# namascar/correlation

Hardware: AMD Instinct MI355X
Metric: correlation-point-iterations/sec (higher is better)
Workload: dtype f32

## Files before the change

### correlation_amd/csrc/lk_device.hpp

```cpp
#pragma once
#include <hip/hip_runtime.h>
#include <stdint.h>

#include "../../include/lk_engine.h"

struct LkLevelView {
  const uint8_t *und;
  const uint8_t *def;
  const float2 *xy;
  const float2 *xy_eval;
  const uint32_t *off;
  const int4 *rect;
  int urows, ucols;
  int drows, dcols;
};

struct LkHandoff {
  float p[6];
  int level;
  int level_old;
  int reached;
  uint32_t n_evals, n_sample_evals, n_point_iters;
};

struct LkSeqFrame {
  const uint8_t *und[LK_MAX_LEVELS];
  const uint8_t *def[LK_MAX_LEVELS];
};
constexpr int kLkSeqChainWords = 16;

constexpr int kLkMaxTeam = 256;
constexpr int kLkMidWords = 32;

struct LkSolveArgs {
  const LkLevelView *lv;
  const float2 *center;
  const float *guess;
  lk_result *result;
  float *last_p;
  float *last_eval_p;
  uint32_t *stats;
  const uint32_t *order;
  int team_w;
  int team_min_samples;
  float *team_partials;
  uint32_t *team_arrivals;
  int team_fault;
  int eval_cap;
  int finisher;
  int resume;
  uint32_t *ill_list;
  uint32_t *ill_count;
  uint32_t *mid_state;
  uint32_t *finish_list;
  uint32_t *finish_count;
  LkHandoff *handoff;
  uint32_t *queue;
  int n_sectors;
  int chunk;
  int align;
  int solo;
  int safe;
  int reference_order;
  int mark_stale;
  int persistent;
  int rows_used;
  int starved_max;
  int keep_sums;
  int gpu_share;
  int slots_permille;
  int py_start, py_step, py_stop;
  float precision;
  int max_iters;
  int seq_frames;
  int seq_velocity;
  int seq_stride;
  const LkSeqFrame *seq_img;
  unsigned long long *seq_chain;
  const float *seq_prev_p;
  float *seq_prev_p_out;
  float *seq_guess_out;
  uint32_t *seq_flags;
  const uint32_t *seq_gate;
  int seq_fault;
};

struct LkRoiSector {
  int kind;
  int x0, y0, x1, y1;
  float cx, cy, ri2, ro2;
  float q00x, q01x, q10x, q11x, q00y, q01y, q10y, q11y;
  int as;
  int flat_begin, flat_count;
};
struct LkRoiFlat {
  float ls, li, rs, ri;
  int j0, j1;
  int row_begin;
};
constexpr int kLkRoiTile = 1024;

struct LkRewarpArgs {
  const float2 *src_xy;
  const uint32_t *src_off;
  const int4 *src_rect;
  const uint32_t *dst_off;
  float2 *dst_xy;
  const float2 *center;
  const float *p;
  const float2 *offset;
  int n_sectors;
  uint32_t total;
  int rows;
};

struct LkAppendArgs {
  int sector, n_levels;
  int keep_state;
  float2 center;
  float2 *d_center;
  float *d_guess, *d_last_p, *d_prev_p, *d_last_eval_p;
  lk_result *d_result;
  uint32_t *d_stats;
  int4 rect[LK_MAX_LEVELS];
  uint32_t off_end[LK_MAX_LEVELS];
  int4 *d_rect[LK_MAX_LEVELS];
  uint32_t *d_off[LK_MAX_LEVELS];
};

struct LkEvalArgs {
  const LkLevelView *lv;
  const float2 *center;
  int sector, level;
  float p[6];
  float *out;
  int ref_threads;
};

struct LkGuessSearchArgs {
  const uint8_t *und, *def;
  int urows, ucols, drows, dcols;
  const float2 *xy;
  const uint32_t *off;
  const int4 *rect;
  float *guess;
  float *prev_p;
  lk_guess_match *match;
  int n_sectors, level, radius, has_v, min_samples;
  float min_score;
  int win_bytes;
};
constexpr int kLkGsThreads = 256;
constexpr int kLkGsChunk = 1024;

struct LkBackwardArgs {
  const LkLevelView *lv;
  const float2 *center;
  const float *guess;
  lk_result *result;
  float *last_p;
  float *last_eval_p;
  uint32_t *stats;
  const uint32_t *order;
  float4 *tpl;
  const uint32_t *tpl_base;
  int n_sectors;
  int py_start, py_step, py_stop;
// ... 16 lines not shown
```

### correlation_amd/csrc/lk_engine.cpp

```cpp
#include "lk_compose.hpp"
#include "lk_device.hpp"
#include "lk_internal.hpp"
#include "lk_roi.hpp"

#include <rocprofiler-sdk-roctx/roctx.h>

#include <algorithm>
#include <chrono>
#include <climits>
#include <cstdio>
#include <cstdlib>
#include <cstring>
#include <functional>
#include <mutex>
#include <string>
#include <thread>
#include <vector>

hipError_t lk_launch_solve(const LkSolveArgs &a, int model, int interp, int group, hipStream_t st);
hipError_t lk_launch_solve_seq(const LkSolveArgs &a, int model, int interp, int group, int flavour, hipStream_t st);
hipError_t lk_launch_eval(const LkEvalArgs &a, int model, int interp, int group, hipStream_t st);
hipError_t lk_launch_solve_only(int n, const float *d_in, float *d_out, hipStream_t st);
hipError_t lk_launch_step_compare(int n, const float *d_in, float *d_out, hipStream_t st);
hipError_t lk_launch_reduce_compare(int n, int wide, const float *d_in, float *d_out, hipStream_t st);
// ... 862 lines not shown
    for (int k = w; k < count; k += workers) {
      const float *q = params + 6 * (size_t)k;
      HostSector &s = e->hs[(size_t)(first_sector + k)];
      s.xy.clear();
      s.is_rect = false;
      s.flats.clear();
      s.fresh = true;
      if (!lkroi::annular_geometry(q[0], q[1], q[2], q[3], q[4], q[5], as, s.ag)) {
        empty[(size_t)w] = 1;
        continue;
      }
      s.lazy = 1;
      if (on_host) {
        s.realize();
        if (s.xy.empty()) {
          empty[(size_t)w] = 1;
          continue;
        }
      }
      s.has_center = false;
      s.set = true;
    }
  };
  std::vector<std::thread> th;
  for (int w = 1; w < workers; ++w)
    th.emplace_back(work, w);
  work(0);
  for (std::thread &t : th)
    t.join();
  for (int v : empty)
    if (v)
      return e->fail(LK_ERROR_BAD_DOMAIN, "lk_set_sectors_annular: empty sector");
  return LK_ERROR_NONE;
}

int lk_set_sector_blob(lk_engine *e, int sector, const float *contour_xy, int n_vertices) {
  if (!e)
    return LK_ERROR_BAD_DOMAIN;
  HostSector *s = sector_slot(e, sector);
  if (!s || !contour_xy)
    return e->fail(LK_ERROR_BAD_DOMAIN, "lk_set_sector_blob: bad arguments");
  s->xy.clear();
  s->is_rect = false;
  s->flats.clear();
  s->lazy = 0;
  if (host_roi()) {
    if (!lkroi::BlobPolygon::inside_points(contour_xy, n_vertices, s->xy) || s->xy.empty()) {
      s->set = false;
      return e->fail(LK_ERROR_BAD_DOMAIN, "lk_set_sector_blob: contour is not a simple polygon");
    }
    lkroi::mean_center(s->xy.data(), (int)(s->xy.size() / 2), s->cx, s->cy);
  } else {
    if (!lkroi::BlobPolygon::flat_triangles(contour_xy, n_vertices, s->flats) || s->flats.empty()) {
      s->set = false;
      return e->fail(LK_ERROR_BAD_DOMAIN, "lk_set_sector_blob: contour is not a simple polygon");
    }
    s->lazy = 2;
  }
  s->has_center = false;
  s->set = true;
  return LK_ERROR_NONE;
}

int lk_set_sector_points(lk_engine *e, int sector, const float *xy, int n, int use_center, float cx,
                         float cy) {
  if (!e)
    return LK_ERROR_BAD_DOMAIN;
  HostSector *s = sector_slot(e, sector);
  if (!s || !xy || n < 1)
    return e->fail(LK_ERROR_BAD_DOMAIN, "lk_set_sector_points: bad arguments");
  s->xy.assign(xy, xy + 2 * (size_t)n);
  s->is_rect = false;
  if (use_center) {
    s->cx = cx;
    s->cy = cy;
  } else {
    lkroi::mean_center(xy, n, s->cx, s->cy);
  }
  s->has_center = use_center != 0;
  s->set = true;
  return LK_ERROR_NONE;
}

static int starved_max(const lk_engine *e) { return e->starved_max >= 0 ? e->starved_max : 2 * e->P; }
static int refresh_starved(lk_engine *e) {
  const int S = (int)e->h_class.size();
  {
    const char *f = std::getenv("LK_STARVED_MAX");
    e->starved_max = f ? std::atoi(f) : -1;
  }
  for (int c = 0; c < kNumClasses; ++c)
    e->class_starved[c] = false;
  if (const char *f = std::getenv("LK_FORCE_SAFE"))
    e->force_safe = std::atoi(f) != 0;
  const int l = e->cfg.py_stop;
  bool any_starved = false;
  for (int s = 0; s < S; ++s) {
    const int4 r = e->h_rect[l][(size_t)s];
    const int n = r.z > 0 ? r.w : (int)(e->h_off[l][(size_t)s + 1] - e->h_off[l][(size_t)s]);
    if (n <= starved_max(e))
      e->class_starved[e->h_class[(size_t)s]] = any_starved = true;
  }
  if (any_starved) {
    HIPCHK(e->d_finish_list.ensure((size_t)S));
    HIPCHK(e->d_finish_count.ensure(kNumClasses));
  }
  return LK_ERROR_NONE;
}

static int level0_count(const lk_engine *e, int s) {
  const int4 r = e->h_rect[0][(size_t)s];
  return r.z > 0 ? r.w : (int)(e->h_off[0][(size_t)s + 1] - e->h_off[0][(size_t)s]);
}

static int build_lists_roi_device(lk_engine *e, const std::vector<int> &levels) {
  Range range_("lk:roi masks");
  const int S = (int)e->hs.size();
  hipStream_t st = e->stream;
  std::vector<LkRoiSector> sec((size_t)S);
  std::vector<LkRoiFlat> flats;
  std::vector<uint32_t> tile_begin((size_t)S + 1, 0u);
  uint64_t tiles = 0;
  bool non_negative = true;
  for (int s = 0; s < S; ++s) {
    const HostSector &h = e->hs[(size_t)s];
    LkRoiSector &q = sec[(size_t)s];
    std::memset(&q, 0, sizeof(q));
    tile_begin[(size_t)s] = (uint32_t)tiles;
    if (h.lazy == 1) {
      const lkroi::AnnularGeometry &g = h.ag;
      q.kind = 0;
      q.x0 = g.x0, q.y0 = g.y0, q.x1 = g.x1, q.y1 = g.y1;
      q.cx = g.cx, q.cy = g.cy, q.ri2 = g.ri2, q.ro2 = g.ro2;
      q.q00x = g.q00x, q.q01x = g.q01x, q.q10x = g.q10x, q.q11x = g.q11x;
      q.q00y = g.q00y, q.q01y = g.q01y, q.q10y = g.q10y, q.q11y = g.q11y;
      q.as = g.as;
      const int64_t w = std::max(0, g.x1 - g.x0), hh = std::max(0, g.y1 - g.y0);
      if (w * hh >= (int64_t)1 << 31)
        return e->fail(LK_ERROR_BAD_DOMAIN, "lk_commit_sectors: annular sector bounding box too large");
      q.x1 = q.x0 + (int)w, q.y1 = q.y0 + (int)hh;
      non_negative = non_negative && std::max((float)q.x0, g.cx - g.ro) >= 0.f && std::max((float)q.y0, g.cy - g.ro) >= 0.f &&
                     q.x1 < (1 << 15) && q.y1 < (1 << 15);
      tiles += (uint64_t)((w * hh + kLkRoiTile - 1) / kLkRoiTile);
    } else {
      q.kind = 1;
      q.flat_begin = (int)flats.size();
      q.flat_count = (int)h.flats.size();
      uint64_t rows = 0;
      for (const lkroi::BlobPolygon::Flat &f : h.flats) {
        LkRoiFlat d;
        d.ls = f.ls, d.li = f.li, d.rs = f.rs, d.ri = f.ri, d.j0 = f.j0, d.j1 = f.j1;
        d.row_begin = (int)rows;
        rows += (uint64_t)(f.j1 - f.j0);
        flats.push_back(d);
        for (int j : {f.j0, f.j1 - 1}) {
          const float a = std::ceil(f.ls * (float)j + f.li), b = std::ceil(f.rs * (float)j + f.ri);
          non_negative = non_negative && j >= 0 && j < (1 << 15) && a >= 0.f && b < 32768.f;
        }
      }
      tiles += rows;
    }
    if (tiles >= (uint64_t)1 << 31)
      return e->fail(LK_ERROR_BAD_DOMAIN, "lk_commit_sectors: region of interest too large for the device mask");
  }
  tile_begin[(size_t)S] = (uint32_t)tiles;
  const uint32_t n_tiles = (uint32_t)tiles;
  if (n_tiles == 0)
    return e->fail(LK_ERROR_BAD_DOMAIN, "lk_commit_sectors: empty region of interest");
  HIPCHK(e->d_roi_sectors.ensure((size_t)S));
  HIPCHK(e->d_roi_flats.ensure(flats.size() + 1));
  HIPCHK(e->d_roi_tile_begin.ensure((size_t)S + 1));
  HIPCHK(hipMemcpyAsync(e->d_roi_sectors.p, sec.data(), (size_t)S * sizeof(LkRoiSector), hipMemcpyHostToDevice, st));
// ... 1023 lines not shown
  if (!xy || cap <= 0)
    return LK_ERROR_NONE;
  HIPCHK(hipSetDevice(e->cfg.device));
  HIPCHK(e->d_warp.ensure(2 * (size_t)n));
  HIPCHK(hipMemcpyAsync(e->d_warp.p + n, pts.data(), 2 * sizeof(float) * (size_t)n, hipMemcpyHostToDevice,
                        e->stream));
  float pp[6] = {0, 0, 0, 0, 0, 0};
  for (int i = 0; i < e->P; ++i)
    pp[i] = p[i];
  HIPCHK(hipMemcpyAsync(e->d_scratch.p, pp, sizeof(pp), hipMemcpyHostToDevice, e->stream));
  HIPCHK(lk_launch_warp_points(e->d_warp.p + n, n, e->h_center[2 * (size_t)sector],
                               e->h_center[2 * (size_t)sector + 1], e->cfg.fitting_model, e->d_scratch.p,
                               e->d_warp.p, e->stream));
  HIPCHK(hipMemcpyAsync(xy, e->d_warp.p, 2 * sizeof(float) * (size_t)std::min(n, cap),
                        hipMemcpyDeviceToHost, e->stream));
  HIPCHK(hipStreamSynchronize(e->stream));
  return LK_ERROR_NONE;
}

static int refresh_level_views(lk_engine *e) {
  if (!e->committed)
    return e->fail(LK_ERROR_BAD_DOMAIN, "sectors are not committed (call lk_commit_sectors)");
  if (e->recommit_pending) {
    e->recommit_pending = false;
    int rc = commit_impl(e, true);
    if (rc)
      return rc;
  }
  const DevImage &u = e->img[LK_IMG_UND], &d = e->img[LK_IMG_DEF];
  if (!u.valid || !d.valid)
    return e->fail(LK_ERROR_BAD_DOMAIN, "undeformed and deformed images must be set before correlating");
  if (!e->lv_dirty)
    return LK_ERROR_NONE;
  for (int l = 0; l < LK_MAX_LEVELS; ++l) {
    LkLevelView &v = e->h_lv[l];
    std::memset(&v, 0, sizeof(v));
    if (l > e->cfg.py_stop)
      continue;
    v.und = u.lvl[l];
    v.def = d.lvl[l];
    v.xy = e->d_xy[l].p;
    v.xy_eval = e->eval_lists && !e->batch_invariant ? e->d_xy_eval[l].p : nullptr;
    v.off = e->d_off[l].p;
    v.rect = e->d_rect[l].p;
    v.urows = u.rows >> l;
    v.ucols = u.cols >> l;
    v.drows = d.rows >> l;
    v.dcols = d.cols >> l;
  }
  if (!e->d_lv.p || std::memcmp(e->h_lv, e->h_lv_sent, sizeof(e->h_lv)) != 0) {
    HIPCHK(e->d_lv.ensure(LK_MAX_LEVELS));
    HIPCHK(lk_launch_set_views(e->h_lv, e->d_lv.p, e->stream));
    std::memcpy(e->h_lv_sent, e->h_lv, sizeof(e->h_lv));
  }
  e->lv_dirty = false;
  return LK_ERROR_NONE;
}

static bool safe_flavour(const lk_engine *e) { return e->force_safe || e->batch_invariant; }

static LkSolveArgs base_args(lk_engine *e, const float *d_guess, lk_result *d_result) {
  LkSolveArgs a{};
  a.lv = e->d_lv.p;
  a.center = e->d_center.p;
  a.guess = d_guess;
  a.result = d_result;
  a.last_p = e->d_last_p.p;
  a.last_eval_p = e->d_last_eval_p.p;
  a.stats = e->d_stats.p;
  a.py_start = e->cfg.py_start;
  a.py_step = e->cfg.py_step;
  a.py_stop = e->cfg.py_stop;
  a.precision = e->cfg.precision;
  a.max_iters = e->cfg.max_iters;
  a.solo = e->batch_invariant ? 0 : 1;
  a.gpu_share = e->pairs_in_flight;
  static const int align = [] {
    const char *f = std::getenv("LK_ALIGN");
    return f ? std::atoi(f) : 1;
  }();
  a.align = align;
  const char *ks = std::getenv("LK_KEEP_SUMS");
  a.keep_sums = ks ? (std::atoi(ks) != 0 ? 1 : 0) : 1;
  a.starved_max = starved_max(e);
  return a;
}

static int launch_starved(lk_engine *e, LkSolveArgs &a, int c, int first, hipStream_t st) {
  a.handoff = e->d_handoff.p;
  a.eval_cap = e->eval_cap > 0 ? e->eval_cap : 0;
  a.mid_state = e->d_mid.p;
  a.finish_list = e->d_finish_list.p + first;
  a.finish_count = e->d_finish_count.p + c;
  if (a.eval_cap > 0)
    HIPCHK(hipMemsetAsync(a.finish_count, 0, sizeof(uint32_t), st));
  HIPCHK(lk_launch_solve(a, e->cfg.fitting_model, e->cfg.interpolation, 1, st));
  if (a.eval_cap > 0) {
    LkSolveArgs f = a;
    f.finisher = 1;
    f.safe = 1;
    f.align = 0;
    HIPCHK(lk_launch_solve(f, e->cfg.fitting_model, e->cfg.interpolation, 16, st));
  }
  a.eval_cap = 0;
  return LK_ERROR_NONE;
}

static int launch_groups(lk_engine *e, LkSolveArgs &a, int group, int c, int first, hipStream_t st) {
  static const bool ill_env = [] { const char *f = std::getenv("LK_ILL_PASS"); return f ? std::atoi(f) != 0 : true; }();
  const bool with_ill_pass = !a.safe && ill_env;
  if (with_ill_pass) {
    a.mid_state = e->d_mid.p;
    a.ill_list = e->d_ill_list.p + first;
    a.ill_count = e->d_ill_count.p + c;
  }
  HIPCHK(lk_launch_solve(a, e->cfg.fitting_model, e->cfg.interpolation, group, st));
  if (with_ill_pass) {
    LkSolveArgs r = a;
    r.resume = 1;
    r.safe = 1;
    r.ill_list = nullptr;
    r.ill_count = nullptr;
    r.finish_list = a.ill_list;
    r.finish_count = a.ill_count;
    r.team_w = 0;
    r.handoff = nullptr;
    r.queue = a.queue + 3;
    HIPCHK(lk_launch_solve(r, e->cfg.fitting_model, e->cfg.interpolation, 16, st));
  }
  return LK_ERROR_NONE;
}

static int team_fault_hook() {
  const char *f = std::getenv("LK_TEAM_FAULT");
  return f ? std::atoi(f) : 0;
}
static std::mutex g_team_mu;
static hipEvent_t g_team_done[64] = {};

static int stale_iterations(lk_engine *e, lk_result *d_result, int n) {
  if (!e->d_stale.p) {
    HIPCHK(e->d_stale.ensure(2));
    HIPCHK(hipMemsetAsync(e->d_stale.p, 0, 2 * sizeof(int), e->stream));
  }
  HIPCHK(lk_launch_stale_iterations(d_result, n, e->d_stale.p + e->stale_par, e->d_stale.p + (e->stale_par ^ 1), e->stream));
  e->stale_par ^= 1;
  return LK_ERROR_NONE;
}

static const int kBwGroups[3] = {16, 64, 512};
static int bw_tables(lk_engine *e) {
  if (!e->bw_dirty && e->h_bw_base.size() == (size_t)e->S)
    return LK_ERROR_NONE;
  const int S = e->S;
  e->h_bw_order.clear();
  e->h_bw_base.assign((size_t)S, 0u);
  size_t total = 0;
  for (int s = 0; s < S; ++s) {
    e->h_bw_base[(size_t)s] = (uint32_t)total;
    total += (size_t)level0_count(e, s);
  }
  if (total > 0xffffffffull)
    return e->fail(LK_ERROR_BAD_DOMAIN, "backward update: more than 2^32 level-0 samples");
  for (int g = 0; g < 3; ++g) {
    e->bw_begin[g] = (int)e->h_bw_order.size();
    for (int s = 0; s < S; ++s)
// ... 1208 lines not shown
```

### correlation_amd/csrc/lk_kernels.hip

```cpp
#include "lk_device.hpp"
#include "lk_internal.hpp"

#include <float.h>
#include <stdlib.h>

#include <atomic>

#include "lk_solver_common.hpp"

namespace {

struct LevelCtx {
  gptr<uint8_t> und, def;
  gptr<f32x2> xy;
  int rx, ry, rw;
  int n;
  int urows, ucols, drows, dcols;
  float cx, cy, scaling;
  float inv_w;
};

__device__ __forceinline__ float row16_sum(float v) {
  v = dpp_add<0xB1>(v);
  v = dpp_add<0x4E>(v);
// ... 844 lines not shown
#pragma unroll
    for (int r = 0; r < 4; ++r) {
      used[r] += trips * cnt[r];
      rem[r] -= trips * cnt[r];
    }
  }
  tot0 += acc0;
  if constexpr (TWO)
    tot1 += acc1;
  __builtin_amdgcn_fence(__ATOMIC_RELEASE, "wavefront");
  float *back = tile + row * 32;
  if (g < N)
    back[g] = tot0;
  if constexpr (TWO)
    if (g + 16 < N)
      back[g + 16] = tot1;
  __builtin_amdgcn_fence(__ATOMIC_RELEASE, "wavefront");
  __builtin_amdgcn_wave_barrier();
  __builtin_amdgcn_fence(__ATOMIC_ACQUIRE, "wavefront");
#pragma unroll
  for (int v = 0; v < N; ++v)
    S.v[v] = back[v];
  __builtin_amdgcn_fence(__ATOMIC_RELEASE, "wavefront");
  return ((bad_sectors >> row) & 1u) != 0u;
}


enum : int { PH_EVAL0 = 0, PH_TENT = 1, PH_REEVAL = 2, PH_FETCH = 3, PH_EXIT = 4, PH_WAIT = 5 };
constexpr int kStaleIterations = (int)0x80000000;

struct Cold {
  float lg_p[6];
  float lambda, lg_chi, c0x, c0y;
  int iteration, reached, error, level, level_old, s, use_saved;
  uint32_t n_evals, n_sample_evals, n_point_iters;
  uint32_t n_ill;
  int sums_kept;
};
constexpr int kColdWords = sizeof(Cold) / 4;
static_assert(kColdWords % 4 == 2 && kColdWords + 7 <= kLkMidWords, "slot = 128-bit words + one 64-bit; the parked-sector record holds it");

template <bool IN_LDS, bool VEC = false> struct ColdStore {
  Cold reg;
  __device__ __forceinline__ Cold load(const uint32_t *slot) const {
    if constexpr (IN_LDS && VEC) {
      Cold k;
      uint4 *w = reinterpret_cast<uint4 *>(&k);
      const uint4 *src = reinterpret_cast<const uint4 *>(slot);
#pragma unroll
      for (int i = 0; i < kColdWords / 4; ++i)
        w[i] = src[i];
      *reinterpret_cast<uint2 *>(w + kColdWords / 4) = *reinterpret_cast<const uint2 *>(src + kColdWords / 4);
      return k;
    } else if constexpr (IN_LDS) {
      Cold k;
      uint32_t *w = reinterpret_cast<uint32_t *>(&k);
#pragma unroll
      for (int i = 0; i < kColdWords; ++i)
        w[i] = slot[i];
      return k;
    } else {
      return reg;
    }
  }
  __device__ __forceinline__ void store(uint32_t *slot, const Cold &k) {
    if constexpr (IN_LDS && VEC) {
      const uint4 *w = reinterpret_cast<const uint4 *>(&k);
      uint4 *dst = reinterpret_cast<uint4 *>(slot);
#pragma unroll
      for (int i = 0; i < kColdWords / 4; ++i)
        dst[i] = w[i];
      *reinterpret_cast<uint2 *>(dst + kColdWords / 4) = *reinterpret_cast<const uint2 *>(w + kColdWords / 4);
    } else if constexpr (IN_LDS) {
      const uint32_t *w = reinterpret_cast<const uint32_t *>(&k);
#pragma unroll
      for (int i = 0; i < kColdWords; ++i)
        slot[i] = w[i];
    } else {
      reg = k;
    }
  }
};

#ifndef LK_MIN_WAVES
#define LK_MIN_WAVES 1
#endif
#ifndef LK_MIN_WAVES_512
#define LK_MIN_WAVES_512 1
#endif
#ifdef LK_TRACE
__device__ unsigned long long g_lk_trace[8 * 16384];
#endif
template <int MODEL, int INTERP, int GROUP, int THREADS, bool SAFE, bool REF = false, bool SEQ = false>
__global__ void __launch_bounds__(THREADS, (THREADS == 64 ? (GROUP == 16 && !SAFE && !REF ? 4 : LK_MIN_WAVES) : THREADS == 512 ? LK_MIN_WAVES_512 : 1)) lk_solve_kernel(LkSolveArgs a) {
  static_assert(!REF || (SAFE && ((THREADS == kWave && (GROUP == 16 || GROUP == kWave)) || (THREADS == 512 && GROUP == 512))), "reference-order instances");
  static_assert(!SEQ || (THREADS == kWave && GROUP >= 16 && GROUP <= kWave), "frame-pipelined instances: one wavefront per workgroup");
  if constexpr (SEQ) {
    if (a.seq_gate && __hip_atomic_load(a.seq_gate, __ATOMIC_RELAXED, __HIP_MEMORY_SCOPE_AGENT) == 0u)
      return;
  }
  constexpr int P = n_params(MODEL);
  using SumsT = Sums<P>;
  constexpr bool COLD_IN_LDS = GROUP > 1 && GROUP <= kWave;
  constexpr bool STARVED = GROUP == 1;
  constexpr bool SCATTER = GROUP == 32 && !SAFE && !REF && !SEQ && P == 6;
  const bool finisher = !REF && SAFE && GROUP == 16 && a.finisher != 0;
  constexpr bool ORD = REF;
  constexpr bool ordered_all = REF;
  const bool starved = STARVED || finisher || ordered_all;
  constexpr int RED_WORDS = GROUP > kWave ? (THREADS / kWave) * (SumsT::N + 1) + 1 : 1;
  __shared__ float lds[RED_WORDS];
  constexpr bool FLAT = REF && GROUP == 16;
  constexpr bool ORD_WG = REF && GROUP == 512;
  __shared__ __attribute__((aligned(16))) float ord_lds[FLAT ? flat_tile_floats<SumsT::N>() : ORD_WG ? wg_ord_floats<SumsT::N>() : ORD ? ord_floats<SumsT::N, (ORD && !ORD_WG) ? GROUP : 16>() : 4];
  __shared__ __attribute__((aligned(16))) OrdCtx ord_ctx[FLAT ? 4 : 1];
  constexpr bool KEEP_SUMS = GROUP == 1 || GROUP == 16;
  constexpr int kSlotWordsRaw = kColdWords + (KEEP_SUMS && COLD_IN_LDS ? SumsT::N : 0);
  constexpr int kSlotWords = GROUP == 32 ? (kSlotWordsRaw + 3) & ~3 : kSlotWordsRaw;
  __shared__ __attribute__((aligned(16))) uint32_t cold_lds[COLD_IN_LDS ? (THREADS / GROUP) * kSlotWords : 4];
  uint32_t *cold_slot = cold_lds + (COLD_IN_LDS ? ((int)threadIdx.x / GROUP) * kSlotWords : 0);
  ColdStore<COLD_IN_LDS, GROUP == 32> cold;
  __shared__ float kept_lds[KEEP_SUMS && !COLD_IN_LDS ? SumsT::N * THREADS : 1];
  auto keep_sums = [&](const SumsT &v) {
    if constexpr (KEEP_SUMS && COLD_IN_LDS) {
#pragma unroll
      for (int i = 0; i < SumsT::N; ++i)
        cold_slot[kColdWords + i] = __float_as_uint(v.v[i]);
    } else if constexpr (KEEP_SUMS) {
#pragma unroll
      for (int i = 0; i < SumsT::N; ++i)
        kept_lds[i * THREADS + (int)threadIdx.x] = v.v[i];
    }
  };
  auto kept_sums = [&](SumsT &v) {
    if constexpr (KEEP_SUMS && COLD_IN_LDS) {
#pragma unroll
      for (int i = 0; i < SumsT::N; ++i)
        v.v[i] = __uint_as_float(cold_slot[kColdWords + i]);
    } else if constexpr (KEEP_SUMS) {
#pragma unroll
      for (int i = 0; i < SumsT::N; ++i)
        v.v[i] = kept_lds[i * THREADS + (int)threadIdx.x];
    }
  };

  __shared__ LkLevelView lv_lds[LK_MAX_LEVELS];
  {
    constexpr int WORDS = (int)(sizeof(LkLevelView) / 4);
    const uint32_t *src = reinterpret_cast<const uint32_t *>(a.lv);
    uint32_t *dst = reinterpret_cast<uint32_t *>(lv_lds);
    for (int i = (int)threadIdx.x; i < WORDS * (a.py_stop + 1); i += THREADS)
      dst[i] = src[i];
    __syncthreads();
  }
  float p[6];
#pragma unroll
  for (int i = 0; i < 6; ++i)
    p[i] = 0.f;
  const float min_lambda = 1e-9f, max_lambda = 1e9f;
  bool first_fetch = true;
  int phase = PH_FETCH;
  int cur_level = 0;
  LevelCtx c{};
  SumsT S;
  bool wide = false;
  int width = 16;
  int cur_frame = 0;
  uint32_t wait_spins = 0;
  constexpr bool UNIFIED = SEQ && !REF && SAFE && GROUP == 16;
  TeamCtx team;
  if constexpr (GROUP == 512) {
    if (a.team_w > 1) {
      team.w = a.team_w;
      team.rank = (int)blockIdx.x % a.team_w;
      team.slot = (int)blockIdx.x / a.team_w;
      team.partials = a.team_partials;
      team.arrivals = a.team_arrivals;
      team.n_slots = a.n_sectors;
      team.fault = a.team_fault;
      team.stride = a.team_w;
      if (a.team_min_samples > 0 && team.slot < a.n_sectors) {
        const int sector = a.order ? (int)a.order[team.slot] : team.slot;
        const LkLevelView lv0 = lv_lds[0];
        const int4 rc = lv0.rect[sector];
        const int n0 = rc.z > 0 ? rc.w : (int)(lv0.off[sector + 1] - lv0.off[sector]);
        int w = (n0 + a.team_min_samples - 1) / a.team_min_samples;
        w = w < 1 ? 1 : (w > a.team_w ? a.team_w : w);
        if (team.rank >= w)
          return;
        team.w = w;
      }
    }
  }

  auto level_count = [&](int level, int sector) -> int {
    const LkLevelView lv = lv_lds[level];
    const int4 rc = lv.rect[sector];
    return rc.z > 0 ? rc.w : (int)(lv.off[sector + 1] - lv.off[sector]);
  };

  auto hand_over = [&](const Cold &k) {
    LkHandoff h;
#pragma unroll
    for (int i = 0; i < 6; ++i)
// ... 132 lines not shown
  const unsigned long long tr_c0 = __builtin_amdgcn_s_memtime();
  unsigned long long tr_eval = 0, tr_steps = 0, tr_solve = 0, tr_fetch = 0, tr_post = 0;
  unsigned long long tr_idle = 0, tr_sleeps = 0;
#endif
  for (;;) {
    bool may_fetch = true;
    if constexpr (GROUP > 1 && GROUP < kWave) {
      if (a.align && a.persistent && !FLAT)
        may_fetch = __ballot(phase < PH_FETCH) == 0ull;
    }
    if constexpr (GROUP == 16) {
      if (width != 16 && a.align && a.persistent && may_fetch) {
        width = 16;
        cold_slot = cold_lds + ((int)threadIdx.x / GROUP) * kSlotWords;
      }
    }
#ifdef LK_TRACE_FINE
    const unsigned long long tr_f0 = __builtin_amdgcn_s_memtime();
#endif
    if (phase == PH_FETCH && may_fetch)
     for (;;) {
      int slot = 0;
      const int n_parked = (finisher || a.resume) ? (int)*(const volatile uint32_t *)a.finish_count : 0;
      if (!a.persistent) {
        const int wg_slot = ((int)blockIdx.x & 7) * a.chunk + ((int)blockIdx.x >> 3);
        slot = first_fetch ? wg_slot * (THREADS / GROUP) + (int)threadIdx.x / GROUP : a.n_sectors;
        if constexpr (FLAT) {
          if (a.rows_used > 0 && a.rows_used < 4)
            slot = (first_fetch && (int)threadIdx.x / GROUP < a.rows_used) ? wg_slot * a.rows_used + (int)threadIdx.x / GROUP : a.n_sectors;
        }
        if (GROUP == 512 && a.team_w > 1)
          slot = first_fetch ? team.slot : a.n_sectors;
        first_fetch = false;
      } else if constexpr (GROUP > kWave) {
        __syncthreads();
        if (threadIdx.x == 0)
          reinterpret_cast<int *>(lds)[RED_WORDS - 1] = (int)atomicAdd(a.queue, 1u);
        __syncthreads();
        slot = reinterpret_cast<int *>(lds)[RED_WORDS - 1];
      } else {
        if ((int)threadIdx.x % GROUP == 0)
          slot = (int)atomicAdd(a.queue, 1u);
        slot = __shfl(slot, ((int)threadIdx.x & 63) & ~(GROUP - 1), 64);
      }
      steps = 0;
      if constexpr (SEQ) {
        if (slot < a.n_sectors * a.seq_frames) {
          Cold k{};
          cur_frame = slot / a.n_sectors;
          const int pos = slot - cur_frame * a.n_sectors;
          k.s = a.order ? (int)a.order[pos] : pos;
          const float2 c0 = a.center[k.s];
          k.c0x = c0.x;
          k.c0y = c0.y;
          k.use_saved = 1;
          k.level = a.py_stop;
          k.level_old = 0;
          cold.store(cold_slot, k);
          phase = PH_WAIT;
        } else {
          phase = PH_EXIT;
        }
      } else if (finisher || a.resume) {
        if (a.resume && !finisher && (int)threadIdx.x % GROUP == 0 &&
            slot == n_parked + (int)gridDim.x * (THREADS / GROUP) - 1) {
          *a.finish_count = 0u;
          *a.queue = 0u;
        }
        if (slot < n_parked) {
          Cold k;
          const int s_idx = (int)a.finish_list[slot];
          const uint32_t *m = a.mid_state + (size_t)s_idx * kLkMidWords;
          uint32_t *w = reinterpret_cast<uint32_t *>(&k);
#pragma unroll
          for (int i = 0; i < kColdWords; ++i)
            w[i] = m[i];
#pragma unroll
          for (int i = 0; i < 6; ++i)
            p[i] = __uint_as_float(m[kColdWords + i]);
          phase = (int)m[kColdWords + 6];
          k.sums_kept = 0;
          level_context(k);
          cold.store(cold_slot, k);
        } else {
          phase = PH_EXIT;
        }
      } else if (slot < a.n_sectors) {
        Cold k{};
        k.s = a.order ? (int)a.order[slot] : slot;
        const float2 c0 = a.center[k.s];
        k.c0x = c0.x;
        k.c0y = c0.y;
        k.use_saved = 1;
        if (!STARVED && a.handoff) {
          const LkHandoff h = a.handoff[k.s];
#pragma unroll
          for (int i = 0; i < 6; ++i)
            p[i] = i < P ? h.p[i] : 0.f;
          k.level = h.level;
          k.level_old = h.level_old;
          k.reached = h.reached;
          k.n_evals = h.n_evals;
          k.n_sample_evals = h.n_sample_evals;
          k.n_point_iters = h.n_point_iters;
        } else {
#pragma unroll
          for (int i = 0; i < 6; ++i)
            p[i] = i < P ? a.guess[(size_t)k.s * 6 + i] : 0.f;
          k.level = a.py_stop;
          k.level_old = 0;
        }
        if (k.level < a.py_start) {
          if (!a.persistent || STARVED)
            phase = PH_EXIT;
        } else if (STARVED && level_count(k.level, k.s) > a.starved_max) {
          hand_over(k);
        } else {
          enter_level(k);
          cold.store(cold_slot, k);
        }
      } else {
        phase = PH_EXIT;
      }
      const bool all_drew_nothing = __ballot(phase != PH_FETCH) == 0ull;
      if (phase == PH_FETCH && all_drew_nothing)
        continue;
      break;
     }
#if defined(LK_TRACE_FINE) && !defined(LK_TRACE_TRANS)
    tr_fetch += __builtin_amdgcn_s_memtime() - tr_f0;
#endif
    if constexpr (SEQ) {
      if (phase == PH_WAIT) {
        Cold k = cold.load(cold_slot);
        bool ready = true;
        float g[6];
#pragma unroll
        for (int i = 0; i < 6; ++i)
          g[i] = 0.f;
        if (cur_frame == 0) {
#pragma unroll
          for (int i = 0; i < P; ++i)
            g[i] = a.guess[(size_t)k.s * 6 + i];
        } else {
          const unsigned long long *ch = a.seq_chain + (size_t)k.s * kLkSeqChainWords;
          const unsigned long long *chr = ch + (size_t)((cur_frame - 1) & 1) * 8, *chq = ch + (size_t)(cur_frame & 1) * 8;
          float r[P], q[P];
#pragma unroll
          for (int i = 0; i < P; ++i) {
            const unsigned long long x = __hip_atomic_load(chr + i, __ATOMIC_RELAXED, __HIP_MEMORY_SCOPE_AGENT);
            ready = ready && (uint32_t)(x >> 32) == (uint32_t)cur_frame;
            r[i] = __uint_as_float((uint32_t)x);
            q[i] = r[i];
          }
          if (a.seq_velocity) {
            if (cur_frame == 1) {
#pragma unroll
              for (int i = 0; i < P; ++i)
                q[i] = a.seq_prev_p[(size_t)k.s * 6 + i];
            } else {
#pragma unroll
              for (int i = 0; i < P; ++i) {
                const unsigned long long x = __hip_atomic_load(chq + i, __ATOMIC_RELAXED, __HIP_MEMORY_SCOPE_AGENT);
                ready = ready && (uint32_t)(x >> 32) == (uint32_t)(cur_frame - 1);
                q[i] = __uint_as_float((uint32_t)x);
              }
            }
          }
#pragma unroll
          for (int i = 0; i < P; ++i)
            g[i] = a.seq_velocity ? r[i] + (r[i] - q[i]) : r[i];
          if (ready && cur_frame == a.seq_frames - 1 && a.seq_prev_p_out && (int)threadIdx.x % GROUP == 0) {
#pragma unroll
            for (int i = 0; i < 6; ++i)
              a.seq_prev_p_out[(size_t)k.s * 6 + i] = i < P ? r[i] : 0.f;
          }
        }
        if (ready) {
#pragma unroll
          for (int i = 0; i < 6; ++i)
            p[i] = g[i];
          if (a.seq_guess_out && (int)threadIdx.x % GROUP == 0) {
#pragma unroll
            for (int i = 0; i < 6; ++i)
              a.seq_guess_out[((size_t)cur_frame * (size_t)a.seq_stride + (size_t)k.s) * 6 + i] = g[i];
          }
          enter_level(k);
          cold.store(cold_slot, k);
        }
      }
    }
    bool active = phase < PH_FETCH;
    if constexpr (SEQ) {
      const unsigned long long waiting = __ballot(phase == PH_WAIT);
      if (__ballot(active) == 0ull && waiting != 0ull) {
        ++wait_spins;
        const bool give_up = wait_spins > (1u << 20);
        if (give_up || (wait_spins & 255u) == 0u) {
          if (give_up || __hip_atomic_load(a.seq_flags, __ATOMIC_RELAXED, __HIP_MEMORY_SCOPE_AGENT) != 0u) {
            if (((int)threadIdx.x & 63) == 0)
              __hip_atomic_store(a.seq_flags, 1u, __ATOMIC_RELAXED, __HIP_MEMORY_SCOPE_AGENT);
            return;
          }
        }
#ifdef LK_TRACE
        ++tr_sleeps;
#endif
        __builtin_amdgcn_s_sleep(16);
        continue;
      }
      if (waiting != ~0ull)
        wait_spins = 0;
#ifdef LK_TRACE
      tr_idle += (unsigned long long)(__builtin_popcountll(~__ballot(active)) / GROUP);
#endif
    }
    if constexpr (GROUP >= kWave) {
      if (!active)
        break;
    } else {
      const unsigned long long act = __ballot(active);
      if (act == 0ull)
        break;
      if constexpr (GROUP == 32) {
        const bool lo = (uint32_t)act != 0u, hi = (uint32_t)(act >> 32) != 0u;
        if (a.solo && !wide && lo != hi && __ballot(phase == PH_EXIT) == ~act) {
          auto take = [&](auto &v) {
            const auto other = __shfl_xor(v, 32, 64);
            if (!active)
              v = other;
          };
#pragma unroll
          for (int i = 0; i < 6; ++i)
            take(p[i]);
          take(c.rx), take(c.ry), take(c.rw), take(c.n);
          take(c.urows), take(c.ucols), take(c.drows), take(c.dcols);
          take(c.scaling), take(c.cx), take(c.cy), take(c.inv_w);
          auto take_ptr = [&](auto &ptr) {
            unsigned long long bits = (unsigned long long)(uintptr_t)ptr;
            uint32_t lo32 = (uint32_t)bits, hi32 = (uint32_t)(bits >> 32);
            take(lo32), take(hi32);
            ptr = (decltype(+ptr))(uintptr_t)(((unsigned long long)hi32 << 32) | lo32);
          };
          take_ptr(c.und), take_ptr(c.def), take_ptr(c.xy);
          take(phase);
          take(cur_level);
          if (!active)
            cold_slot = cold_lds + (((int)threadIdx.x / GROUP) ^ 1) * kSlotWords;
          active = true;
          wide = true;
        }
      }
    }
    if constexpr (GROUP == 16) {
      const unsigned long long act = __ballot(active);
      const bool idle_ok = (a.align && a.persistent) || __ballot(phase == PH_EXIT) == ~act;
      if (a.solo && width < 64 && idle_ok && !finisher && !ordered_all) {
        const unsigned rows = ((act & 0xffffull) ? 1u : 0u) | ((act & 0xffff0000ull) ? 2u : 0u) |
                              ((act & 0xffff00000000ull) ? 4u : 0u) | ((act & 0xffff000000000000ull) ? 8u : 0u);
        const unsigned sect = width == 16 ? rows : ((rows & 3u) ? 1u : 0u) | ((rows & 12u) ? 4u : 0u);
        const int n_sect = __builtin_popcount(sect);
        const int new_width = n_sect == 1 ? 64 : (n_sect == 2 && width == 16) ? 32 : width;
        if (new_width != width) {
          const int first = __builtin_ctz(sect), last = 31 - __builtin_clz(sect);
          const int lane = (int)threadIdx.x & 63;
          const int src_row = (new_width == 64 || lane < 32) ? first : last;
          const int src_lane = src_row * 16 + (lane & 15);
          auto take = [&](auto &v) { v = __shfl(v, src_lane, 64); };
#pragma unroll
          for (int i = 0; i < 6; ++i)
            take(p[i]);
          take(c.rx), take(c.ry), take(c.rw), take(c.n);
          take(c.urows), take(c.ucols), take(c.drows), take(c.dcols);
          take(c.scaling), take(c.cx), take(c.cy);
          auto take_ptr = [&](auto &ptr) {
            unsigned long long bits = (unsigned long long)(uintptr_t)ptr;
            uint32_t lo32 = (uint32_t)bits, hi32 = (uint32_t)(bits >> 32);
            take(lo32), take(hi32);
            ptr = (decltype(+ptr))(uintptr_t)(((unsigned long long)hi32 << 32) | lo32);
          };
          take_ptr(c.und), take_ptr(c.def), take_ptr(c.xy);
          take(phase);
          take(cur_level);
          int slot_idx = (int)(cold_slot - cold_lds);
          take(slot_idx);
          cold_slot = cold_lds + slot_idx;
          active = phase < PH_FETCH;
          width = new_width;
        }
      }
    }
    if constexpr (GROUP > 1 && GROUP < kWave) {
      if (a.align && !FLAT) {
        int wave_level = -1;
        for (int L = a.py_stop; L >= a.py_start && wave_level < 0; L -= a.py_step)
          if (__ballot(active && cur_level == L) != 0ull)
            wave_level = L;
        if (active && cur_level < wave_level)
          active = false;
      }
    }
    LevelCtx ce = c;
    if (!active)
      ce.n = 0;
    bool row_ordered = finisher;
    if constexpr (UNIFIED) {
      const bool ord = active && c.n <= a.starved_max;
      const bool any_plain = __ballot(active && !ord) != 0ull;
      row_ordered = active ? ord : !any_plain;
    }
#ifdef LK_TRACE
    const unsigned long long tr_e0 = __builtin_amdgcn_s_memtime();
#endif
    bool err;
    if constexpr (FLAT) {
      err = a.reference_order > 1 ? evaluate_ordered_flat<MODEL, INTERP, true>(ce, p, S, ord_lds, ord_ctx, a.reference_order)
                                  : evaluate_ordered_flat<MODEL, INTERP, false>(ce, p, S, ord_lds, ord_ctx, 1);
    } else if constexpr (ORD_WG) {
      if (team.w > 1) {
        const int T = team.w, cq = ce.n / T, cr = ce.n - cq * T;
        const int first = team.rank * cq + (team.rank < cr ? team.rank : cr), count = cq + (team.rank < cr ? 1 : 0);
        err = evaluate_ordered_wg<MODEL, INTERP, false>(ce, p, S, ord_lds, 1, first, count);
        err = team_all_to_all(S, err, lds, &team);
      } else {
        err = a.reference_order > 1 ? evaluate_ordered_wg<MODEL, INTERP, true>(ce, p, S, ord_lds, a.reference_order, 0, ce.n)
                                    : evaluate_ordered_wg<MODEL, INTERP, false>(ce, p, S, ord_lds, 1, 0, ce.n);
      }
    } else if constexpr (ORD) {
      err = a.reference_order > 1 ? evaluate_ordered<MODEL, INTERP, GROUP, true>(ce, p, S, ord_lds, a.reference_order)
                                  : evaluate_ordered<MODEL, INTERP, GROUP, false>(ce, p, S, ord_lds, 1);
    } else {
      err = evaluate<MODEL, INTERP, GROUP, THREADS, SCATTER>(ce, p, S, lds, &team, wide, row_ordered, GROUP == 16 ? width : 0);
    }
#ifdef LK_TRACE
    tr_eval += __builtin_amdgcn_s_memtime() - tr_e0;
    ++tr_steps;
#endif
#ifdef LK_TRACE_FINE
    const unsigned long long tr_p0 = __builtin_amdgcn_s_memtime();
#endif
    if constexpr (GROUP == 512) {
      if (team.timed_out && team.w > 1) {
        if (team.rank != 0)
          return;
        team.w = 1;
        team.timed_out = false;
        phase = PH_FETCH;
        first_fetch = true;
        continue;
      }
    }
    if (active) {
      Cold k = cold.load(cold_slot);
      float evaluated[6];
#pragma unroll
      for (int i = 0; i < 6; ++i)
        evaluated[i] = p[i];
      const int evaluated_level = k.level;
      ++k.n_evals;
      k.n_sample_evals += (uint32_t)c.n;
      bool level_end = false, iter_start = false, finished = false, handed = false;
      if (err) {
        k.error = LK_ERROR_INTERPOLATION_OUT_OF_IMAGE;
        if (phase == PH_EVAL0) {
          ++k.n_point_iters;
          translate<P>(p, k.level, 0);
          finished = true;
        } else {
          level_end = true;
        }
      } else {
        const float chi = S.v[SumsT::N - 1] * c.scaling;
        float lam_use = phase == PH_TENT ? fmaxf(k.lambda * 0.4f, min_lambda) : k.lambda;
        bool redo = false;
        if constexpr (KEEP_SUMS) {
          if (phase == PH_TENT && k.sums_kept != 0 && !(chi <= k.lg_chi)) {
            const float delta_chi = __builtin_fabsf((k.lg_chi - chi) / (fmaxf(k.lg_chi, chi) + a.precision));
            const float lambda_new = fminf(k.lambda * 10.0f, max_lambda);
            redo = !(delta_chi < a.precision) && !(k.iteration + 1 > a.max_iters || lambda_new >= max_lambda);
            if constexpr (!SAFE && !STARVED) {
              if (redo && a.ill_list) {
                float q[6];
#pragma unroll
                for (int i = 0; i < 6; ++i)
                  q[i] = p[i];
                redo = damped_step<P, false>(S, lam_use, c.scaling, q, false);
              }
            }
            if (redo) {
              k.lambda = lambda_new;
              k.use_saved = 0;
              ++k.iteration;
              k.reached = k.iteration;
              ++k.n_point_iters;
              lam_use = lambda_new;
#pragma unroll
              for (int i = 0; i < P; ++i)
                p[i] = k.lg_p[i];
            }
          }
          if (phase != PH_TENT || chi <= k.lg_chi)
            keep_sums(S);
          if (redo)
            kept_sums(S);
        }
        float tent[P];
#pragma unroll
        for (int i = 0; i < P; ++i)
          tent[i] = p[i];
#ifdef LK_TRACE
        const unsigned long long tr_s0 = __builtin_amdgcn_s_memtime();
#endif
        const bool step_starved = starved || (UNIFIED && row_ordered);
        bool wc;
        if constexpr (SCATTER)
          wc = damped_step_scattered(S.v[0], S.v[1], lam_use, c.scaling, p);
        else
          wc = damped_step<P, SAFE || STARVED>(S, lam_use, c.scaling, p, step_starved, nullptr, SAFE && GROUP >= 16 && GROUP <= kWave);
#ifdef LK_TRACE
        tr_solve += __builtin_amdgcn_s_memtime() - tr_s0;
#endif
        if (!wc && !step_starved)
          ++k.n_ill;
        if constexpr (SEQ && !SAFE) {
          if (!wc && (int)threadIdx.x % GROUP == 0)
            __hip_atomic_store(a.seq_flags + 1, 1u, __ATOMIC_RELAXED, __HIP_MEMORY_SCOPE_AGENT);
        }
        bool ill_parked = false;
        if constexpr (!SAFE && !STARVED) {
          if (!wc && a.ill_list) {
#pragma unroll
            for (int i = 0; i < P; ++i)
              p[i] = tent[i];
            if (redo) {
              phase = PH_REEVAL;
// ... 1749 lines not shown
```

Before: 461.7 million.

## Keep hot LM iteration state in registers instead of reloading cold slot

Adds a register-resident HotState (lambda, lg_chi, iteration, counters) for SCATTER kernels and a new per-step path that updates only a few cold-slot words in place. The full Cold struct is loaded and stored only on error, ill-conditioning or level end, which cuts per-iteration LDS/memory traffic. Hot state is carried through wave compaction via take(). It also adds an LK_STEP_STATE env switch back to the old path and a 'none' option for LK_STARVED_MAX. The cost is extra register pressure and a duplicated control path that must stay in sync with the original.

```diff
diff --git a/correlation_amd/csrc/lk_device.hpp b/correlation_amd/csrc/lk_device.hpp
--- a/correlation_amd/csrc/lk_device.hpp
+++ b/correlation_amd/csrc/lk_device.hpp
@@ -83,6 +83,7 @@
   uint32_t *seq_flags;
   const uint32_t *seq_gate;
   int seq_fault;
+  int slot_step;
 };
 
 struct LkRoiSector {
diff --git a/correlation_amd/csrc/lk_engine.cpp b/correlation_amd/csrc/lk_engine.cpp
--- a/correlation_amd/csrc/lk_engine.cpp
+++ b/correlation_amd/csrc/lk_engine.cpp
@@ -968,12 +968,13 @@
   return LK_ERROR_NONE;
 }
 
-static int starved_max(const lk_engine *e) { return e->starved_max >= 0 ? e->starved_max : 2 * e->P; }
+constexpr int kStarvedNone = -2;
+static int starved_max(const lk_engine *e) { return e->starved_max == kStarvedNone ? -1 : e->starved_max >= 0 ? e->starved_max : 2 * e->P; }
 static int refresh_starved(lk_engine *e) {
   const int S = (int)e->h_class.size();
   {
     const char *f = std::getenv("LK_STARVED_MAX");
-    e->starved_max = f ? std::atoi(f) : -1;
+    e->starved_max = !f ? -1 : std::strcmp(f, "none") == 0 ? kStarvedNone : std::atoi(f) >= 0 ? std::atoi(f) : -1;
   }
   for (int c = 0; c < kNumClasses; ++c)
     e->class_starved[c] = false;
@@ -2163,6 +2164,8 @@
   a.align = align;
   const char *ks = std::getenv("LK_KEEP_SUMS");
   a.keep_sums = ks ? (std::atoi(ks) != 0 ? 1 : 0) : 1;
+  const char *ss = std::getenv("LK_STEP_STATE");
+  a.slot_step = ss && std::atoi(ss) == 0 ? 1 : 0;
   a.starved_max = starved_max(e);
   return a;
 }
diff --git a/correlation_amd/csrc/lk_kernels.hip b/correlation_amd/csrc/lk_kernels.hip
--- a/correlation_amd/csrc/lk_kernels.hip
+++ b/correlation_amd/csrc/lk_kernels.hip
@@ -950,6 +950,24 @@
   }
 };
 
+template <bool ON> struct HotState {
+  __device__ __forceinline__ void take(const Cold &) {}
+  __device__ __forceinline__ void give(Cold &) const {}
+};
+template <> struct HotState<true> {
+  float lambda = 0.f, lg_chi = 0.f;
+  int iteration = 0;
+  uint32_t n_evals = 0u, n_sample_evals = 0u, n_point_iters = 0u;
+  __device__ __forceinline__ void take(const Cold &k) {
+    lambda = k.lambda, lg_chi = k.lg_chi, iteration = k.iteration;
+    n_evals = k.n_evals, n_sample_evals = k.n_sample_evals, n_point_iters = k.n_point_iters;
+  }
+  __device__ __forceinline__ void give(Cold &k) const {
+    k.lambda = lambda, k.lg_chi = lg_chi, k.iteration = iteration;
+    k.n_evals = n_evals, k.n_sample_evals = n_sample_evals, k.n_point_iters = n_point_iters;
+  }
+};
+
 #ifndef LK_MIN_WAVES
 #define LK_MIN_WAVES 1
 #endif
@@ -988,6 +1006,7 @@
   __shared__ __attribute__((aligned(16))) uint32_t cold_lds[COLD_IN_LDS ? (THREADS / GROUP) * kSlotWords : 4];
   uint32_t *cold_slot = cold_lds + (COLD_IN_LDS ? ((int)threadIdx.x / GROUP) * kSlotWords : 0);
   ColdStore<COLD_IN_LDS, GROUP == 32> cold;
+  HotState<SCATTER> hot;
   __shared__ float kept_lds[KEEP_SUMS && !COLD_IN_LDS ? SumsT::N * THREADS : 1];
   auto keep_sums = [&](const SumsT &v) {
     if constexpr (KEEP_SUMS && COLD_IN_LDS) {
@@ -1286,6 +1305,7 @@
           k.sums_kept = 0;
           level_context(k);
           cold.store(cold_slot, k);
+          hot.take(k);
         } else {
           phase = PH_EXIT;
         }
@@ -1322,6 +1342,7 @@
         } else {
           enter_level(k);
           cold.store(cold_slot, k);
+          hot.take(k);
         }
       } else {
         phase = PH_EXIT;
@@ -1449,6 +1470,10 @@
           take_ptr(c.und), take_ptr(c.def), take_ptr(c.xy);
           take(phase);
           take(cur_level);
+          if constexpr (SCATTER) {
+            take(hot.lambda), take(hot.lg_chi), take(hot.iteration);
+            take(hot.n_evals), take(hot.n_sample_evals), take(hot.n_point_iters);
+          }
           if (!active)
             cold_slot = cold_lds + (((int)threadIdx.x / GROUP) ^ 1) * kSlotWords;
           active = true;
@@ -1554,7 +1579,114 @@
         continue;
       }
     }
-    if (active) {
+    if constexpr (SCATTER) {
+      if (active && a.slot_step == 0) {
+        constexpr int W_LG_P = (int)(offsetof(Cold, lg_p) / 4), W_REACHED = (int)(offsetof(Cold, reached) / 4);
+        constexpr int W_USE_SAVED = (int)(offsetof(Cold, use_saved) / 4), W_N_ILL = (int)(offsetof(Cold, n_ill) / 4);
+        static_assert(W_LG_P == 0, "lg_p: one 128-bit and one 64-bit access at the head of the slot");
+        float evaluated[6];
+#pragma unroll
+        for (int i = 0; i < 6; ++i)
+          evaluated[i] = p[i];
+        const int evaluated_level = cur_level;
+        ++hot.n_evals;
+        hot.n_sample_evals += (uint32_t)c.n;
+        bool level_end = false, finished = false, maxed = false, ill = false;
+        if (!err) {
+          const float chi = S.v[SumsT::N - 1] * c.scaling;
+          const bool eval0 = phase == PH_EVAL0, tent = phase == PH_TENT;
+          const float lam_down = fmaxf(hot.lambda * 0.4f, min_lambda);
+          const float lam_use = tent ? lam_down : hot.lambda;
+          const bool accept = eval0 || chi <= hot.lg_chi;
+          const float delta_chi = __builtin_fabsf((hot.lg_chi - chi) / (fmaxf(hot.lg_chi, chi) + a.precision));
+          const bool conv = tent && delta_chi < a.precision;
+#ifdef LK_TRACE
+          const unsigned long long tr_s0 = __builtin_amdgcn_s_memtime();
+#endif
+          const bool wc = damped_step_scattered(S.v[0], S.v[1], lam_use, c.scaling, p);
+#ifdef LK_TRACE
+          tr_solve += __builtin_amdgcn_s_memtime() - tr_s0;
+#endif
+          if (!wc && a.ill_list) {
+            ill = true;
+          } else {
+            if (!wc)
+              ++cold_slot[W_N_ILL];
+            if (phase == PH_REEVAL) {
+              phase = PH_TENT;
+            } else {
+              if (tent && accept) {
+                *reinterpret_cast<uint4 *>(cold_slot) = make_uint4(__float_as_uint(evaluated[0]), __float_as_uint(evaluated[1]),
+                                                                   __float_as_uint(evaluated[2]), __float_as_uint(evaluated[3]));
+                *reinterpret_cast<uint2 *>(cold_slot + 4) = make_uint2(__float_as_uint(evaluated[4]), __float_as_uint(evaluated[5]));
+              }
+              hot.lambda = eval0 ? hot.lambda : accept ? lam_down : fminf(hot.lambda * 10.0f, max_lambda);
+              hot.lg_chi = accept ? chi : hot.lg_chi;
+              hot.iteration = eval0 ? 1 : conv ? hot.iteration : hot.iteration + 1;
+              hot.n_point_iters += eval0 ? 1u : 0u;
+              cold_slot[W_USE_SAVED] = accept ? 1u : 0u;
+              maxed = !conv && (hot.iteration > a.max_iters || hot.lambda >= max_lambda);
+              level_end = conv || maxed;
+              if (!level_end) {
+                cold_slot[W_REACHED] = (uint32_t)hot.iteration;
+                ++hot.n_point_iters;
+                phase = accept ? PH_TENT : PH_REEVAL;
+                if (!accept) {
+#pragma unroll
+                  for (int i = 0; i < P; ++i)
+                    p[i] = __uint_as_float(cold_slot[W_LG_P + i]);
+                }
+              }
+            }
+          }
+        }
+        if (err || ill || level_end) {
+          Cold k = cold.load(cold_slot);
+          hot.give(k);
+          if (err) {
+            k.error = LK_ERROR_INTERPOLATION_OUT_OF_IMAGE;
+            if (phase == PH_EVAL0) {
+              ++k.n_point_iters;
+              translate<P>(p, k.level, 0);
+              finished = true;
+            } else {
+              level_end = true;
+            }
+          }
+          if (ill) {
+            ++k.n_ill;
+#pragma unroll
+            for (int i = 0; i < P; ++i)
+              p[i] = evaluated[i];
+            --k.n_evals;
+            k.n_sample_evals -= (uint32_t)c.n;
+            k.sums_kept = 0;
+            park(k, a.ill_list, a.ill_count);
+          } else {
+            if (maxed)
+              k.error = LK_ERROR_CORRELATION_MAX_ITERS_REACHED;
+            if (level_end) {
+              k.level_old = k.level;
+              k.level -= a.py_step;
+              if (k.level < a.py_start) {
+                translate<P>(p, k.level_old, 0);
+                finished = true;
+              } else {
+                enter_level(k);
+              }
+            }
+            if (finished) {
+              translate<P>(evaluated, evaluated_level, 0);
+              finish_sector(k, evaluated);
+            } else {
+              cold.store(cold_slot, k);
+              hot.take(k);
+            }
+          }
+        }
+      }
+    }
+    if (active && (!SCATTER || a.slot_step != 0)) {
       Cold k = cold.load(cold_slot);
       float evaluated[6];
 #pragma unroll
```

After: 479.3 million (median of 6 runs). +3.8%, better.
